# nebula-beta/MonocularSfM

Hardware: AMD Instinct MI355X
Metric: descriptor-pairs/sec (and image-pairs/sec); match-index bit-parity vs CPU (higher is better)
Workload: dtype f32

## Files before the change

### monocularsfm_amd/csrc/msfm_prefilter.hip.h

```cpp
#pragma once
#include "msfm_kernels.hip.h"

namespace msfm {

constexpr float kEpsRel = 1.5e-3f;
constexpr float kEpsAbs = 1.0e-6f;
constexpr float kF16Safe = 6.0e4f;

constexpr int kPfRB = 2;
constexpr int kPfWaveRows = 32 * kPfRB;
constexpr int kPfWaves = 8;
constexpr int kPfWgRows = kPfWaves * kPfWaveRows;
constexpr int kPfThreads = 64 * kPfWaves;
constexpr int kPfBT = 64;
constexpr int kPfRowHalfs = 136;
constexpr int kPfRowBytes = kPfRowHalfs * 2;
constexpr int kPfTileBytes = kPfBT * kPfRowBytes;
constexpr int kPfTilePieces = kPfTileBytes / 1024;
constexpr int kPfRing = 4;
constexpr int kPfColClasses = 4;
constexpr int kPfCandBuf = 256;
constexpr int kPfLdsBytes = kPfRing * kPfTileBytes + kPfWaves * kPfRing * 64 * 4 + kPfWaves * kPfCandBuf * 8 +
                            2 * kPfBT * kPfColClasses * 4;
static_assert(kPfTileBytes % 1024 == 0 && kPfTilePieces == 17, "tile = 17 DMA pieces");

typedef _Float16 h8 __attribute__((ext_vector_type(8)));
typedef float f16v __attribute__((ext_vector_type(16)));

struct PfPair {
    const _Float16* a_h;
    const _Float16* b_h;
    const _Float16* const* a_rows;
    const float* a_nrm;
    const float* b_nrm;
    float a_c, b_c;
    float a_nrm_max, b_nrm_max;
    long long tu_off;
    long long tv_off;
    long long cand_off;
    int cand_cap;
    int use;
    int i8;
    int a_h0, b_h0;
    int pad;
    const float* a_err;
    const float* b_err;
    const int* a_n2;
    const int* b_n2;
};

__device__ __forceinline__ void glds_copy_bytes(const void* g, void* lds, int bytes, int tid, int nthreads) {
    const int wave = __builtin_amdgcn_readfirstlane(tid >> 6), lane = tid & 63;
    const char* gp = reinterpret_cast<const char*>(g);
    char* lp = reinterpret_cast<char*>(lds);
#pragma unroll 1
    for (int piece = wave; piece * 1024 < bytes; piece += nthreads / 64)
        __builtin_amdgcn_global_load_lds((const __attribute__((address_space(1))) void*)(gp + piece * 1024 + lane * 16),
                                         (__attribute__((address_space(3))) void*)(lp + piece * 1024), 16, 0, 0);
}

__device__ __forceinline__ void v2_merge(float& s0, float& s1, float b0, float b1) {
    s1 = fminf(fmaxf(s0, b0), fminf(s1, b1));
    s0 = fminf(s0, b0);
}

#include "msfm_sweep.hip.h"
#include "msfm_sweep_i8.hip.h"

struct PruneParams {
    int prune;
    float ratio;
    float max_distance;
};

__device__ __forceinline__ bool pf_dead(float s0, float s1, float nrm, float eps, float other_max, PruneParams pr) {
    if (!pr.prune) return false;
    const float tiny = 1e-5f * (fabsf(s0) + fabsf(s1) + nrm + other_max);
    const float s0lb = fmaxf(s0 - eps - tiny, 0.f);
    const float s1ub = s1 + eps + tiny;
    const float d0lb = sqrtf(s0lb) * (1.f - 1e-6f);
    const bool ratio_fails = pr.ratio > 0.f && d0lb >= pr.ratio * sqrtf(s1ub) * (1.f + 1e-5f);
    const bool too_far = d0lb > pr.max_distance * (1.f + 1e-5f);
    return ratio_fails || too_far;
}

struct PlanPair {
    int fwd_member;
    int rev_member0;
    int rev_bits;
    int pad;
};


struct PlanCounts {
    const PlanPair* pp_plan;
    const int* member_group;
    int* cnt;
    int* gtot;
};

__global__ void pf_thresholds_kernel(const PairDesc* __restrict__ pairs, const PfPair* __restrict__ pf,
                                     const float* __restrict__ rp_s0, const float* __restrict__ rp_s1,
                                     const float* __restrict__ cp_s0, unsigned* __restrict__ colmask,
                                     float* __restrict__ tu, float* __restrict__ tv, PruneParams pr, PlanCounts plan,
                                     int marked ) {
    MSFM_TAIL_PRIO();
    const PairDesc pd = pairs[blockIdx.y];
    const PfPair pp = pf[blockIdx.y];
    if (!pd.valid || !pp.use) return;
    const int e = blockIdx.x * blockDim.x + threadIdx.x;
    bool row_live = false;
    unsigned col_bits = 0;
    const float eps_norm = 4.8828125e-4f * fmaxf(pp.a_c, pp.b_c);
    const float2* cp2 = reinterpret_cast<const float2*>(cp_s0);
    const int* cpk = reinterpret_cast<const int*>(cp_s0);
    const int nb = pd.a_blocks256;
    const bool in_r = e < pd.n1pad, in_c = e < pd.n2pad;
    const int er = in_r ? e : 0, ec = in_c ? e : 0;
    const float ld_rs0 = rp_s0[pd.rp_off + er], ld_rs1 = rp_s1[pd.rp_off + er];
    const float ld_anrm = pp.a_nrm[er], ld_bnrm = pp.b_nrm[ec];
    const float ld_tu = marked ? tu[pp.tu_off + er] : 0.f, ld_tv = marked ? tv[pp.tv_off + ec] : 0.f;
    float2 ld_cp[16];
#pragma unroll
    for (int p = 0; p < 16; ++p) {
        const long long i = pd.cp_off + (long long)min(p, nb - 1) * pd.n2pad + ec;
        ld_cp[p] = pp.i8 ? make_float2(__int_as_float(cpk[i]), 0.f) : cp2[i];
    }
    auto partial16 = [&](int p) -> float2 { return pp.i8 ? i8_cp_unpack(__float_as_int(ld_cp[p].x)) : ld_cp[p]; };
    if (in_r && !(marked && ld_tu == -f_inf())) {
        float s0 = f_inf(), s1 = f_inf();
        v2_merge(s0, s1, ld_rs0, ld_rs1);
        for (int p = 1; p < pd.ranges; ++p) {
            const long long o = pd.rp_off + (long long)p * pd.n1pad + e;
            v2_merge(s0, s1, rp_s0[o], rp_s1[o]);
        }
        const float na = ld_anrm;
        const float eps = pp.i8 ? kI8Eps : kEpsRel * (na + pp.b_nrm_max) + kEpsAbs * (sqrtf(na) + sqrtf(pp.b_nrm_max)) + eps_norm;
        const float slack = pp.i8 ? 2.f * eps : 2.f * eps + 1e-5f * (fabsf(s1) + na + pp.b_nrm_max);
        const bool live = (e < pd.n1) && !pf_dead(s0, s1, na, eps, pp.b_nrm_max, pr);
        tu[pp.tu_off + e] = live ? s1 + slack : -f_inf();
        row_live = live;
    }
    if (in_c && marked && ld_tv == -f_inf()) {
        if (colmask) colmask[pp.tv_off + e] = 0;
    } else if (in_c) {
        float s0 = f_inf(), s1 = f_inf();
        auto partial = [&](long long i) -> float2 { return pp.i8 ? i8_cp_unpack(cpk[i]) : cp2[i]; };
        float bmin[16];
        if (nb <= 16) {
#pragma unroll
            for (int p = 0; p < 16; ++p) {
                bmin[p] = f_inf();
                if (p < nb) {
                    const float2 m = partial16(p);
                    bmin[p] = -2.f * m.x;
                    v2_merge(s0, s1, -2.f * m.x, -2.f * m.y);
                }
            }
        } else {
            for (int p = 0; p < nb; ++p) {
                const float2 m = partial(pd.cp_off + (long long)p * pd.n2pad + e);
                v2_merge(s0, s1, -2.f * m.x, -2.f * m.y);
            }
        }
        const float nb_ = ld_bnrm;
        const float eps = pp.i8 ? kI8Eps : kEpsRel * (nb_ + pp.a_nrm_max) + kEpsAbs * (sqrtf(nb_) + sqrtf(pp.a_nrm_max)) + eps_norm;
        const float slack = pp.i8 ? 2.f * eps : 2.f * eps + 1e-5f * (fabsf(s1) + nb_ + pp.a_nrm_max);
        const bool live = (e < pd.n2) && !pf_dead(s0, s1, nb_, eps, pp.a_nrm_max, pr);
        const float T = live ? s1 + slack : -f_inf();
        tv[pp.tv_off + e] = T;
        if (colmask) {
            const int g = (nb + 31) / 32;
            unsigned mask = 0;
            if (live) {
                if (nb <= 16) {
#pragma unroll
                    for (int p = 0; p < 16; ++p)
                        if (p < nb && bmin[p] <= T) mask |= 1u << p;
                } else {
                    for (int p = 0; p < nb; ++p) {
                        const float smin = -2.f * partial(pd.cp_off + (long long)p * pd.n2pad + e).x;
                        if (smin <= T) mask |= 1u << (p / g);
                    }
                }
            }
            colmask[pp.tv_off + e] = mask;
            col_bits = mask;
        }
    }
    if (plan.pp_plan) {
        const PlanPair pl = plan.pp_plan[blockIdx.y];
        if (pl.fwd_member < 0) return;
        __shared__ int hist[33];
        if (threadIdx.x < 33) hist[threadIdx.x] = 0;
        __syncthreads();
        const unsigned long long rl = __ballot(row_live);
        if ((threadIdx.x & 63) == 0 && rl) atomicAdd(&hist[32], __popcll(rl));
        while (col_bits) {
            const int bit = __builtin_ctz(col_bits);
            col_bits &= col_bits - 1;
            atomicAdd(&hist[bit], 1);
        }
        __syncthreads();
        if (threadIdx.x == 0 && hist[32]) {
            atomicAdd(&plan.cnt[pl.fwd_member], hist[32]);
            atomicAdd(&plan.gtot[plan.member_group[pl.fwd_member]], hist[32]);
        }
        if ((int)threadIdx.x < pl.rev_bits && hist[threadIdx.x]) {
            atomicAdd(&plan.cnt[pl.rev_member0 + threadIdx.x], hist[threadIdx.x]);
            atomicAdd(&plan.gtot[plan.member_group[pl.rev_member0 + threadIdx.x]], hist[threadIdx.x]);
        }
    }
}

struct CandList {
    int pair;
    int mode;
    long long off;
    int cap;
    int pad;
    const int* live_idx;
    const int* row_pair;
    const float* cmp_tu;
    const int* cmp_n2;
    const int* b_n2;
};

__device__ __forceinline__ unsigned long long pf_key(float s, int idx) {
    return ((unsigned long long)__float_as_uint(s) << 32) | (unsigned)idx;
}

constexpr int kExSpan = 256;
constexpr int kExLists = 1024;

template <int N>
__device__ __forceinline__ float pf_row_shl(float v) {
    return __builtin_bit_cast(float, __builtin_amdgcn_update_dpp(0, __builtin_bit_cast(int, v), 0x100 + N, 0xf, 0xf, true));
}

template <int ORDER>
__device__ __forceinline__ float pf_exact_combine(const float (&av)[8], const float (&bv)[8]) {
    if (ORDER == 0) {
        float p = 0.f;
#pragma unroll
        for (int it = 0; it < 8; ++it) {
            const float t = av[it] - bv[it];
            p = (it == 0) ? t * t : p + t * t;
        }
        const float s = ((p + pf_row_shl<4>(p)) + pf_row_shl<8>(p)) + pf_row_shl<12>(p);
        const float u = s + pf_row_shl<2>(s);
        return u + pf_row_shl<1>(u);
    } else if (ORDER == 3) {
        float s = 0.f;
#pragma unroll
        for (int v = 0; v < 4; ++v) {
            const float t0 = av[v] - bv[v];
            const float t1 = av[4 + v] - bv[4 + v];
            const float p = __builtin_fmaf(t1, t1, t0 * t0);
            s = (v == 0) ? p : s + p;
        }
        const float x = s + pf_row_shl<8>(s);
        const float y = x + pf_row_shl<4>(x);
        const float z = y + pf_row_shl<2>(y);
        return z + pf_row_shl<1>(z);
    } else {
        float pa = 0.f, pb = 0.f;
#pragma unroll
        for (int it = 0; it < 4; ++it) {
            const float ta = av[2 * it] - bv[2 * it];
            const float tb = av[2 * it + 1] - bv[2 * it + 1];
            pa = (it == 0) ? ta * ta : __builtin_fmaf(ta, ta, pa);
            pb = (it == 0) ? tb * tb : __builtin_fmaf(tb, tb, pb);
        }
        const float s = ((pa + pf_row_shl<8>(pa)) + pb) + pf_row_shl<8>(pb);
        const float t = s + pf_row_shl<1>(s);
        const float v = t + pf_row_shl<2>(t);
        return v + pf_row_shl<4>(v);
    }
}

__device__ __forceinline__ void pf_fold(unsigned long long* __restrict__ best, unsigned long long* __restrict__ second, long long slot,
                                        unsigned long long key, unsigned long long sb, unsigned long long ss) {
    msfm_fold_key(best + slot, second + slot, key, sb, ss,
                  [](unsigned long long* w, unsigned long long k) -> unsigned long long { return atomicMin(w, k); });
}

template <int ORDER>
__global__ __launch_bounds__(kExSpan) void pf_exact_candidates_kernel(
    const PairDesc* __restrict__ pairs, const CandList* __restrict__ lists, const unsigned long long* __restrict__ cand_count,
    const int2* __restrict__ cand, unsigned long long* __restrict__ best, unsigned long long* __restrict__ second, int n_lists,
    int* __restrict__ cursors , const int* __restrict__ cand_val , int b_h0_unused) {
    MSFM_TAIL_PRIO();
    __shared__ int s_base[kExLists + 1];
    __shared__ int s_part[kExSpan];
    __shared__ const float* s_a[kExSpan];
    __shared__ const float* s_b[kExSpan];
    __shared__ float s_res[kExSpan];
    __shared__ int s_g;
    const int xcd = blockIdx.x & 7, tid = threadIdx.x, sub = tid & 15, grp = tid >> 4;
    const int my_lists = n_lists > xcd ? (n_lists - xcd + 7) / 8 : 0;
    if (tid == 0) s_g = atomicAdd(&cursors[xcd], 1);
    int round_base = 0;
  for (int l0 = 0; l0 < my_lists; l0 += kExLists) {
    const int nl = min(kExLists, my_lists - l0);
    int cnt4[4], mine = 0;
#pragma unroll
    for (int j = 0; j < 4; ++j) {
        const int i = 4 * tid + j;
        int ns = 0;
        if (i < nl) {
            const int lid = xcd + 8 * (l0 + i);
            const int cap = lists[lid].cap;
            const unsigned long long cc = cand_count[lid];
            const int n = (int)(cc < (unsigned long long)cap ? cc : (unsigned long long)cap);
            ns = (n + kExSpan - 1) / kExSpan;
        }
        cnt4[j] = ns;
        mine += ns;
    }
    __syncthreads();
    s_part[tid] = mine;
    __syncthreads();
    for (int d = 1; d < kExSpan; d <<= 1) {
        const int v = tid >= d ? s_part[tid - d] : 0;
        __syncthreads();
        s_part[tid] += v;
        __syncthreads();
    }
    int run = s_part[tid] - mine;
#pragma unroll
    for (int j = 0; j < 4; ++j) {
        s_base[4 * tid + j] = run;
        run += cnt4[j];
    }
    if (tid == kExSpan - 1) s_base[kExLists] = run;
    __syncthreads();
    const int total = s_base[kExLists];
   for (;;) {
    const int g = s_g - round_base;
    if (g >= total) break;
    int lo = 0, hi = kExLists;
    while (hi - lo > 1) {
        const int mid = (lo + hi) >> 1;
        if (s_base[mid] <= g) lo = mid; else hi = mid;
    }
    const int lid = xcd + 8 * (l0 + lo);
    const CandList L = lists[lid];
    const int n = (int)(cand_count[lid] < (unsigned long long)L.cap ? cand_count[lid] : (unsigned long long)L.cap);
    const int c0 = (g - s_base[lo]) * kExSpan, c1 = min(n, c0 + kExSpan);
    const bool live = c0 + tid < c1;
    int2 qt = cand[L.off + (live ? c0 + tid : c0)];
    float s_int = 0.f;
    if (ORDER == 4) {
        const int acc = cand_val[L.off + (live ? c0 + tid : c0)];
        const int C = (int)floorf(fminf(fmaxf(0.5f * L.cmp_tu[qt.x], -5.0e8f), 5.0e8f));
        s_int = (float)(L.cmp_n2[qt.x] + (L.b_n2[qt.y] & 1) - 2 * (acc - C));
    }
    const int pair = L.mode == 0 ? L.pair : L.row_pair[qt.x];
    if (L.mode == 1) qt.x = L.live_idx[qt.x];
    if (L.mode == 2) qt = make_int2(qt.y, L.live_idx[qt.x]);
    const PairDesc* pd = pairs + pair;
    if (ORDER != 4) {
        s_a[tid] = pd->a_rawp + (size_t)qt.x * kDim;
        s_b[tid] = pd->b_rawp + (size_t)qt.y * kDim;
    }
    const long long slot_r = pd->kf_off + qt.x, slot_c = pd->kr_off + qt.y;
    unsigned long long sb_r = ~0ull, ss_r = ~0ull, sb_c = ~0ull, ss_c = ~0ull;
    if (live && L.mode != 2) sb_r = best[slot_r], ss_r = second[slot_r];
    if (live && L.mode != 1) sb_c = best[slot_c], ss_c = second[slot_c];
    __syncthreads();
    int g_next = 0;
    if (tid == 0) g_next = atomicAdd(&cursors[xcd], 1);
    const int n4 = ORDER == 4 ? 0 : (c1 - c0 + 3) & ~3;
    for (int k0 = grp; k0 < n4; k0 += 32) {
        const int k1 = k0 + 16 < n4 ? k0 + 16 : k0;
        const float* a0 = s_a[k0];
        const float* b0 = s_b[k0];
        const float* a1 = s_a[k1];
        const float* b1 = s_b[k1];
        float av0[8], bv0[8], av1[8], bv1[8];
        {
            const float4* pa0 = reinterpret_cast<const float4*>(a0) + sub;
            const float4* pb0 = reinterpret_cast<const float4*>(b0) + sub;
            const float4* pa1 = reinterpret_cast<const float4*>(a1) + sub;
            const float4* pb1 = reinterpret_cast<const float4*>(b1) + sub;
            const float4 x0 = pa0[0], x1 = pa0[16], y0 = pb0[0], y1 = pb0[16];
            const float4 z0 = pa1[0], z1 = pa1[16], w0 = pb1[0], w1 = pb1[16];
            av0[0] = x0.x, av0[1] = x0.y, av0[2] = x0.z, av0[3] = x0.w, av0[4] = x1.x, av0[5] = x1.y, av0[6] = x1.z, av0[7] = x1.w;
            bv0[0] = y0.x, bv0[1] = y0.y, bv0[2] = y0.z, bv0[3] = y0.w, bv0[4] = y1.x, bv0[5] = y1.y, bv0[6] = y1.z, bv0[7] = y1.w;
            av1[0] = z0.x, av1[1] = z0.y, av1[2] = z0.z, av1[3] = z0.w, av1[4] = z1.x, av1[5] = z1.y, av1[6] = z1.z, av1[7] = z1.w;
            bv1[0] = w0.x, bv1[1] = w0.y, bv1[2] = w0.z, bv1[3] = w0.w, bv1[4] = w1.x, bv1[5] = w1.y, bv1[6] = w1.z, bv1[7] = w1.w;
        }
        const float r0 = pf_exact_combine<ORDER>(av0, bv0);
        const float r1 = pf_exact_combine<ORDER>(av1, bv1);
        if (sub == 0) {
            s_res[k0] = r0;
            s_res[k1] = r1;
        }
    }
    if (tid == 0) s_g = g_next;
    __syncthreads();
    if (live) {
        const float res = ORDER == 4 ? s_int : s_res[tid];
        if (res < f_inf()) {
            if (L.mode != 2) pf_fold(best, second, slot_r, pf_key(res, qt.y), sb_r, ss_r);
            if (L.mode != 1) pf_fold(best, second, slot_c, pf_key(res, qt.x), sb_c, ss_c);
        }
    }
   }
    round_base += total;
  }
}

#include "msfm_plan.hip.h"
#include "msfm_q8.hip.h"
#include "msfm_store.hip.h"

__global__ void pf_finalize_kernel(const PairDesc* __restrict__ pairs, const PfPair* __restrict__ pf,
                                   const float* __restrict__ tuv,
                                   const unsigned long long* __restrict__ best, const unsigned long long* __restrict__ second,
                                   int* __restrict__ k_i0, float* __restrict__ k_d0, float* __restrict__ k_d1,
                                   int* __restrict__ fix_count, int4* __restrict__ fix_list, int fix_cap) {
    MSFM_TAIL_PRIO();
    const PairDesc pd = pairs[blockIdx.y];
    const PfPair pp = pf[blockIdx.y];
    if (!pd.valid || !pp.use) return;
    const int e = blockIdx.x * blockDim.x + threadIdx.x;
    for (int dir = 0; dir < 2; ++dir) {
        const int n = dir == 0 ? pd.n1 : pd.n2;
        if (e >= n) continue;
        const long long ko = (dir == 0 ? pd.kf_off : pd.kr_off) + e;
        const bool dead = tuv[ko] == -f_inf();
        const unsigned long long b = dead ? ~0ull : best[ko], s = dead ? ~0ull : second[ko];
        int i0 = -1;
        float d0 = 3.402823466e+38f, d1 = 3.402823466e+38f;
        if (b != ~0ull) { i0 = (int)(unsigned)(b & 0xffffffffu); d0 = sqrtf(__uint_as_float((unsigned)(b >> 32))); }
        if (s != ~0ull) d1 = sqrtf(__uint_as_float((unsigned)(s >> 32)));
        k_i0[ko] = i0;
        k_d0[ko] = d0;
        k_d1[ko] = d1;
        if (i0 >= 0 && d0 == d1) {
            const int slot = atomicAdd(fix_count, 1);
            if (slot < fix_cap) fix_list[slot] = make_int4((int)blockIdx.y, dir, e, 0);
        }
    }
}

}
```

Measured before the change: 5514 billion.

## Bucket-sort exact candidates by query row to reuse A descriptor loads

Within each 256-candidate span, candidates are counting-sorted by query row into LDS using shared-memory atomics and a DPP wave scan, so each 16-lane group processes a contiguous run of candidates that share the same A row. The A descriptor is reloaded only when the row pointer changes, cutting redundant global reads. The best/second words are now read after the distance is computed rather than prefetched up front, and the per-candidate slot is staged in LDS. This adds extra barriers, scan work and LDS per block, and it relies on the DPP scan and the conditional-reload logic being correct for parity.

```diff
diff --git a/monocularsfm_amd/csrc/msfm_prefilter.hip.h b/monocularsfm_amd/csrc/msfm_prefilter.hip.h
--- a/monocularsfm_amd/csrc/msfm_prefilter.hip.h
+++ b/monocularsfm_amd/csrc/msfm_prefilter.hip.h
@@ -232,10 +232,21 @@
 
 constexpr int kExSpan = 256;
 constexpr int kExLists = 1024;
+constexpr int kExBuckets = 512;
 
 template <int N>
 __device__ __forceinline__ float pf_row_shl(float v) {
     return __builtin_bit_cast(float, __builtin_amdgcn_update_dpp(0, __builtin_bit_cast(int, v), 0x100 + N, 0xf, 0xf, true));
+}
+
+__device__ __forceinline__ int pf_wave_scan(int v) {
+    v += __builtin_amdgcn_update_dpp(0, v, 0x111, 0xf, 0xf, true);
+    v += __builtin_amdgcn_update_dpp(0, v, 0x112, 0xf, 0xf, true);
+    v += __builtin_amdgcn_update_dpp(0, v, 0x114, 0xf, 0xf, true);
+    v += __builtin_amdgcn_update_dpp(0, v, 0x118, 0xf, 0xf, true);
+    v += __builtin_amdgcn_update_dpp(0, v, 0x142, 0xa, 0xf, false);
+    v += __builtin_amdgcn_update_dpp(0, v, 0x143, 0xc, 0xf, false);
+    return v;
 }
 
 template <int ORDER>
@@ -296,10 +307,14 @@
     __shared__ const float* s_a[kExSpan];
     __shared__ const float* s_b[kExSpan];
     __shared__ float s_res[kExSpan];
+    __shared__ int s_cnt[ORDER == 4 ? 1 : kExBuckets];
+    __shared__ int s_wtot[kExSpan / 64];
+    __shared__ long long s_slot[kExSpan];
     __shared__ int s_g;
     const int xcd = blockIdx.x & 7, tid = threadIdx.x, sub = tid & 15, grp = tid >> 4;
     const int my_lists = n_lists > xcd ? (n_lists - xcd + 7) / 8 : 0;
     if (tid == 0) s_g = atomicAdd(&cursors[xcd], 1);
+    if (ORDER != 4) s_cnt[2 * tid] = s_cnt[2 * tid + 1] = 0;
     int round_base = 0;
   for (int l0 = 0; l0 < my_lists; l0 += kExLists) {
     const int nl = min(kExLists, my_lists - l0);
@@ -357,54 +372,88 @@
         s_int = (float)(L.cmp_n2[qt.x] + (L.b_n2[qt.y] & 1) - 2 * (acc - C));
     }
     const int pair = L.mode == 0 ? L.pair : L.row_pair[qt.x];
+    const int key_row = qt.x;
     if (L.mode == 1) qt.x = L.live_idx[qt.x];
     if (L.mode == 2) qt = make_int2(qt.y, L.live_idx[qt.x]);
     const PairDesc* pd = pairs + pair;
+    s_slot[tid] = L.mode == 2 ? pd->kr_off + qt.y : pd->kf_off + qt.x;
+    int slot = tid;
     if (ORDER != 4) {
-        s_a[tid] = pd->a_rawp + (size_t)qt.x * kDim;
-        s_b[tid] = pd->b_rawp + (size_t)qt.y * kDim;
-    }
-    const long long slot_r = pd->kf_off + qt.x, slot_c = pd->kr_off + qt.y;
-    unsigned long long sb_r = ~0ull, ss_r = ~0ull, sb_c = ~0ull, ss_c = ~0ull;
-    if (live && L.mode != 2) sb_r = best[slot_r], ss_r = second[slot_r];
-    if (live && L.mode != 1) sb_c = best[slot_c], ss_c = second[slot_c];
+        const int bucket = key_row & (kExBuckets - 1);
+        int arrival = 0;
+        if (live) arrival = atomicAdd(&s_cnt[bucket], 1);
+        const float* ra = pd->a_rawp + (size_t)qt.x * kDim;
+        const float* rb = pd->b_rawp + (size_t)qt.y * kDim;
+        __syncthreads();
+        const int n0 = s_cnt[2 * tid], n1 = s_cnt[2 * tid + 1];
+        const int inc = pf_wave_scan(n0 + n1);
+        if ((tid & 63) == 63) s_wtot[tid >> 6] = inc;
+        __syncthreads();
+        int first = inc - (n0 + n1);
+#pragma unroll
+        for (int w = 0; w < kExSpan / 64 - 1; ++w)
+            if ((tid >> 6) > w) first += s_wtot[w];
+        s_cnt[2 * tid] = first;
+        s_cnt[2 * tid + 1] = first + n0;
+        __syncthreads();
+        if (live) slot = s_cnt[bucket] + arrival;
+        s_a[slot] = L.mode == 2 ? rb : ra;
+        s_b[slot] = L.mode == 2 ? ra : rb;
+    }
     __syncthreads();
     int g_next = 0;
     if (tid == 0) g_next = atomicAdd(&cursors[xcd], 1);
-    const int n4 = ORDER == 4 ? 0 : (c1 - c0 + 3) & ~3;
-    for (int k0 = grp; k0 < n4; k0 += 32) {
-        const int k1 = k0 + 16 < n4 ? k0 + 16 : k0;
-        const float* a0 = s_a[k0];
-        const float* b0 = s_b[k0];
-        const float* a1 = s_a[k1];
-        const float* b1 = s_b[k1];
-        float av0[8], bv0[8], av1[8], bv1[8];
-        {
+    if (ORDER != 4) {
+        s_cnt[2 * tid] = s_cnt[2 * tid + 1] = 0;
+        const int n_span = c1 - c0, share = (n_span + 15) >> 4;
+        const float* a_have = nullptr;
+        float4 k0 = make_float4(0.f, 0.f, 0.f, 0.f), k1 = k0;
+#pragma unroll 1
+        for (int j = 0; j < share; j += 2) {
+            const int i0 = min(grp * share + j, n_span - 1), i1 = min(grp * share + j + (j + 1 < share ? 1 : 0), n_span - 1);
+            const float* a0 = s_a[i0];
+            const float* b0 = s_b[i0];
+            const float* a1 = s_a[i1];
+            const float* b1 = s_b[i1];
             const float4* pa0 = reinterpret_cast<const float4*>(a0) + sub;
             const float4* pb0 = reinterpret_cast<const float4*>(b0) + sub;
             const float4* pa1 = reinterpret_cast<const float4*>(a1) + sub;
             const float4* pb1 = reinterpret_cast<const float4*>(b1) + sub;
-            const float4 x0 = pa0[0], x1 = pa0[16], y0 = pb0[0], y1 = pb0[16];
-            const float4 z0 = pa1[0], z1 = pa1[16], w0 = pb1[0], w1 = pb1[16];
-            av0[0] = x0.x, av0[1] = x0.y, av0[2] = x0.z, av0[3] = x0.w, av0[4] = x1.x, av0[5] = x1.y, av0[6] = x1.z, av0[7] = x1.w;
-            bv0[0] = y0.x, bv0[1] = y0.y, bv0[2] = y0.z, bv0[3] = y0.w, bv0[4] = y1.x, bv0[5] = y1.y, bv0[6] = y1.z, bv0[7] = y1.w;
-            av1[0] = z0.x, av1[1] = z0.y, av1[2] = z0.z, av1[3] = z0.w, av1[4] = z1.x, av1[5] = z1.y, av1[6] = z1.z, av1[7] = z1.w;
-            bv1[0] = w0.x, bv1[1] = w0.y, bv1[2] = w0.z, bv1[3] = w0.w, bv1[4] = w1.x, bv1[5] = w1.y, bv1[6] = w1.z, bv1[7] = w1.w;
-        }
-        const float r0 = pf_exact_combine<ORDER>(av0, bv0);
-        const float r1 = pf_exact_combine<ORDER>(av1, bv1);
-        if (sub == 0) {
-            s_res[k0] = r0;
-            s_res[k1] = r1;
+            const bool new0 = a0 != a_have, new1 = a1 != a0;
+            int take1 = new1;
+            asm volatile("" : "+v"(take1));
+            if (new0) k0 = pa0[0], k1 = pa0[16];
+            float4 z0 = make_float4(0.f, 0.f, 0.f, 0.f), z1 = z0;
+            if (new1) z0 = pa1[0], z1 = pa1[16];
+            const float4 y0 = pb0[0], y1 = pb0[16];
+            const float4 w0 = pb1[0], w1 = pb1[16];
+            const float av0[8] = {k0.x, k0.y, k0.z, k0.w, k1.x, k1.y, k1.z, k1.w};
+            const float bv0[8] = {y0.x, y0.y, y0.z, y0.w, y1.x, y1.y, y1.z, y1.w};
+            const float r0 = pf_exact_combine<ORDER>(av0, bv0);
+            if (take1) k0 = z0, k1 = z1;
+            const float av1[8] = {k0.x, k0.y, k0.z, k0.w, k1.x, k1.y, k1.z, k1.w};
+            const float bv1[8] = {w0.x, w0.y, w0.z, w0.w, w1.x, w1.y, w1.z, w1.w};
+            const float r1 = pf_exact_combine<ORDER>(av1, bv1);
+            if (sub == 0) {
+                s_res[i0] = r0;
+                s_res[i1] = r1;
+            }
+            a_have = a1;
         }
     }
     if (tid == 0) s_g = g_next;
     __syncthreads();
     if (live) {
-        const float res = ORDER == 4 ? s_int : s_res[tid];
+        const float res = ORDER == 4 ? s_int : s_res[slot];
         if (res < f_inf()) {
-            if (L.mode != 2) pf_fold(best, second, slot_r, pf_key(res, qt.y), sb_r, ss_r);
-            if (L.mode != 1) pf_fold(best, second, slot_c, pf_key(res, qt.x), sb_c, ss_c);
+            const long long slot_p = s_slot[tid];
+            const unsigned long long sb_p = best[slot_p], ss_p = second[slot_p];
+            pf_fold(best, second, slot_p, pf_key(res, L.mode == 2 ? qt.x : qt.y), sb_p, ss_p);
+            if (L.mode == 0) {
+                const long long slot_c = pairs[L.pair].kr_off + qt.y;
+                const unsigned long long sb_c = best[slot_c], ss_c = second[slot_c];
+                pf_fold(best, second, slot_c, pf_key(res, qt.x), sb_c, ss_c);
+            }
         }
     }
    }
```

Measured after the change: 5534 billion, median of 4. Within noise of the previous version (+0.4%).
